# samiwilf/torchrec-oldfork

Hardware: AMD Instinct MI355X
Metric: samples/sec Criteo-1TB DLRM batch 65536 (higher is better)
Workload: dtype f32; 1 GPU; DLRM Criteo-1TB shape: 26 tables (177.9M rows, 84.85 GiB fp32, D=128), 13 dense, pooling factor 1, dense 512-256-128, over 1024-1024-512-256-1, fused exact SGD; global_batch=65536, local_batch=65536, parallelism=mp1: 26 table-wise + 0 row-wise + 0 replicated (data-parallel) tables, dense dp1, ids=uniform, distinct_batches=32, seed=0, data_ranks=1

## Files before the change

### include/tbe_hip.h

```cpp
#ifndef TBE_HIP_H_
#define TBE_HIP_H_

#include <stddef.h>
#include <stdint.h>

#ifdef __cplusplus
extern "C" {
#endif

#define TBE_OK 0
#define TBE_ERR_INVALID_ARGUMENT (-1)
#define TBE_ERR_LAUNCH (-2)
#define TBE_ERR_WORKSPACE (-3)
#define TBE_ERR_UNSUPPORTED (-4)

#define TBE_POOL_SUM 0
#define TBE_POOL_MEAN 1
#define TBE_POOL_NONE 2

#define TBE_OPT_EXACT_SGD 0
#define TBE_OPT_EXACT_ROWWISE_ADAGRAD 1
#define TBE_OPT_ADAM 2
#define TBE_OPT_EXACT_ADAGRAD 3
#define TBE_OPT_DENSE_GRAD 100
// ... 199 lines not shown
                                int32_t B, int32_t D_total, int32_t all_multiple_of_4, void* stream);

int tbe_dlrm_interaction_forward_f32(const float* dense, const float* sparse, int32_t B,
                                     int32_t F, int32_t D, float* out, int64_t out_row_stride,
                                     void* stream);
int tbe_dlrm_interaction_backward_f32(const float* dense, const float* sparse,
                                      const float* grad_out, int64_t grad_row_stride, int32_t B, int32_t F, int32_t D,
                                      float* grad_dense, float* grad_sparse, void* stream);

int tbe_dlrm_interaction_gather_forward_f32(const float* dense, const uint64_t* feat_weights, const int64_t* feat_rows,
                                            const int64_t* feat_window, const int64_t* indices, int32_t B, int32_t F,
                                            int32_t D, float* out, int64_t out_row_stride, int32_t* bounds_errors,
                                            void* stream);
int tbe_dlrm_interaction_gather_backward_f32(const float* dense, const uint64_t* feat_weights, const int64_t* feat_rows,
                                             const int64_t* feat_window, const int64_t* indices, const float* grad_out,
                                             int64_t grad_row_stride, int32_t B, int32_t F, int32_t D, float* grad_dense,
                                             float* grad_sparse, int32_t* bounds_errors, void* stream);

size_t tbe_relu_backward_bias_grad_workspace_bytes(int64_t B, int32_t N);
int tbe_relu_backward_bias_grad_f32(const float* grad_out, const float* act, int64_t B, int32_t N,
                                    float* grad_in, float* bias_grad, void* workspace,
                                    size_t workspace_bytes, void* stream);

size_t tbe_weighted_colsum_workspace_bytes(int64_t B, int32_t N);
int tbe_weighted_colsum_f32(const float* x, const float* w, int64_t B, int32_t N, float* out,
                            void* workspace, size_t workspace_bytes, void* stream);

int64_t tbe_colsum_row_blocks(int64_t B, int32_t N);
int tbe_relu_backward_bias_partials_f32(const float* grad_out, const float* act, int64_t B, int32_t N,
                                        float* grad_in, float* partial, size_t partial_bytes, void* stream);
int tbe_weighted_colsum_partials_f32(const float* x, const float* w, int64_t B, int32_t N, float* partial,
                                     size_t partial_bytes, void* stream);

int tbe_multi_chunk_sum_f32(const int64_t* seg_table, int32_t nseg, int64_t max_numel, float* dst, float scale,
                            void* stream);
int tbe_multi_chunk_sum_host_table_f32(const int64_t* host_seg_table, int32_t nseg, int64_t max_numel, float* dst,
                                       float scale, void* stream);

size_t tbe_bce_with_logits_workspace_bytes(void);
int tbe_bce_with_logits_f32(const float* logits, const void* labels, int32_t label_elem_size, int64_t B, float* loss,
                            float* dlogits, void* workspace, size_t workspace_bytes, void* stream);

int tbe_jagged_2d_to_dense_f32(const float* values, const int64_t* offsets, int32_t B,
                               int32_t D, int32_t max_L, float* dense, void* stream);

int tbe_dense_to_jagged_2d_f32(const float* dense, const int64_t* offsets, int32_t B, int32_t D,
// ... 13 lines not shown
```

### torchrec-oldfork_amd/csrc/mlp_epilogue.hip

```cpp
#include <algorithm>
#include <cstring>

#include "common.hpp"

namespace tbe {

__host__ __device__ inline int rows_per_block(int N) { return N >= 512 ? 256 : 64; }

template <int TX>
__global__ __launch_bounds__(256) void drelu_bgrad_kernel(const float* __restrict__ gy, const float* __restrict__ act,
                                                          float* __restrict__ gx, float* __restrict__ partial,
                                                          int64_t B, int N) {
  constexpr int TY = 256 / TX;
  __shared__ float4 red[TY][TX];
  const int tx = threadIdx.x % TX;
  const int ty = threadIdx.x / TX;
  const int col = (blockIdx.x * TX + tx) * 4;
  const int rpb = rows_per_block(N);
  const int64_t row0 = static_cast<int64_t>(blockIdx.y) * rpb;
  const int64_t row1 = min(B, row0 + rpb);
  float4 acc = make_float4(0.f, 0.f, 0.f, 0.f);
  if (col < N) {
#pragma unroll 4
    for (int64_t r = row0 + ty; r < row1; r += TY) {
// ... 45 lines not shown
      const float s = w[r];
      acc.x = fmaf(s, v.x, acc.x);
      acc.y = fmaf(s, v.y, acc.y);
      acc.z = fmaf(s, v.z, acc.z);
      acc.w = fmaf(s, v.w, acc.w);
    }
  }
  red[ty][tx] = acc;
  __syncthreads();
  if (ty == 0 && col < N) {
    float4 s = red[0][tx];
#pragma unroll
    for (int y = 1; y < TY; ++y) {
      const float4 o = red[y][tx];
      s.x += o.x;
      s.y += o.y;
      s.z += o.z;
      s.w += o.w;
    }
    st4(partial + static_cast<int64_t>(blockIdx.y) * N + col, s);
  }
}

__global__ __launch_bounds__(256) void colsum_partials_kernel(const float* __restrict__ partial, int64_t nblocks, int N,
                                                              float* __restrict__ out) {
  __shared__ float red[4][64];
  const int lane = threadIdx.x & 63;
  const int wave = threadIdx.x >> 6;
  const int c = blockIdx.x * 64 + lane;
  float acc = 0.f;
  if (c < N) {
#pragma unroll 8
    for (int64_t rb = wave; rb < nblocks; rb += 4) acc += partial[rb * N + c];
  }
  red[wave][lane] = acc;
  __syncthreads();
  if (wave == 0 && c < N) out[c] = ((red[0][lane] + red[1][lane]) + red[2][lane]) + red[3][lane];
}

struct ChunkSeg {
  const float* src;
  int64_t chunks;
  int64_t numel;
  int64_t dst_off;
};
constexpr int kChunkSegsByValue = 32;
struct ChunkSegs32 {
  ChunkSeg s[kChunkSegsByValue];
};
__device__ __forceinline__ void multi_chunk_sum_body(const ChunkSeg sg, float* __restrict__ dst, float scale);

__global__ __launch_bounds__(256) void multi_chunk_sum_kernel(const ChunkSeg* __restrict__ segs, float* __restrict__ dst,
                                                              float scale) {
  multi_chunk_sum_body(segs[blockIdx.y], dst, scale);
}
__global__ __launch_bounds__(256) void multi_chunk_sum_args_kernel(const ChunkSegs32 segs, float* __restrict__ dst, float scale) {
  multi_chunk_sum_body(segs.s[blockIdx.y], dst, scale);
}

__device__ __forceinline__ void multi_chunk_sum_body(const ChunkSeg sg, float* __restrict__ dst, float scale) {
// ... 196 lines not shown
  }
  TBE_REQUIRE(x && w && workspace, "tbe_weighted_colsum_f32: null pointer");
  TBE_REQUIRE(((reinterpret_cast<uintptr_t>(x) | reinterpret_cast<uintptr_t>(workspace)) & 15) == 0,
              "tbe_weighted_colsum_f32: tensors must be 16-B aligned");
  TBE_REQUIRE(workspace_bytes >= tbe_weighted_colsum_workspace_bytes(B, N), "tbe_weighted_colsum_f32: workspace too small");
  const int rpb = rows_per_block(N);
  const int64_t nrb = (B + rpb - 1) / rpb;
  TBE_REQUIRE(nrb <= 65535, "tbe_weighted_colsum_f32: B=%lld too large", (long long)B);
  float* partial = static_cast<float*>(workspace);
  const int vecs = N / 4;
  if (vecs >= 64) {
    hipLaunchKernelGGL(wcolsum_kernel<64>, dim3((vecs + 63) / 64, static_cast<unsigned>(nrb)), dim3(256), 0, st, x, w, partial, B, N);
  } else if (vecs >= 32) {
    hipLaunchKernelGGL(wcolsum_kernel<32>, dim3((vecs + 31) / 32, static_cast<unsigned>(nrb)), dim3(256), 0, st, x, w, partial, B, N);
  } else {
    hipLaunchKernelGGL(wcolsum_kernel<16>, dim3((vecs + 15) / 16, static_cast<unsigned>(nrb)), dim3(256), 0, st, x, w, partial, B, N);
  }
  TBE_CHECK_LAUNCH("tbe_weighted_colsum_f32");
  hipLaunchKernelGGL(colsum_partials_kernel, dim3((N + 63) / 64), dim3(256), 0, st, partial, nrb, N, out);
  TBE_CHECK_LAUNCH("tbe_weighted_colsum_f32 colsum");
  return TBE_OK;
}


extern "C" int64_t tbe_colsum_row_blocks(int64_t B, int32_t N) {
  if (B <= 0 || N <= 0) return 0;
  const int rpb = rows_per_block(N);
  return (B + rpb - 1) / rpb;
}

extern "C" int tbe_relu_backward_bias_partials_f32(const float* grad_out, const float* act, int64_t B, int32_t N,
                                                   float* grad_in, float* partial, size_t partial_bytes, void* stream) {
  TBE_REQUIRE(B > 0 && N > 0 && (N & 3) == 0, "tbe_relu_backward_bias_partials_f32: B > 0 and N a positive multiple of 4 required");
  TBE_REQUIRE(grad_out && act && grad_in && partial, "tbe_relu_backward_bias_partials_f32: null pointer");
  TBE_REQUIRE(((reinterpret_cast<uintptr_t>(grad_out) | reinterpret_cast<uintptr_t>(act) |
                reinterpret_cast<uintptr_t>(grad_in) | reinterpret_cast<uintptr_t>(partial)) & 15) == 0,
              "tbe_relu_backward_bias_partials_f32: tensors must be 16-B aligned");
  const int64_t nrb = tbe_colsum_row_blocks(B, N);
  TBE_REQUIRE(nrb <= 65535, "tbe_relu_backward_bias_partials_f32: B=%lld too large", (long long)B);
  TBE_REQUIRE(partial_bytes >= static_cast<size_t>(nrb) * N * sizeof(float), "tbe_relu_backward_bias_partials_f32: partial too small");
  hipStream_t st = static_cast<hipStream_t>(stream);
  const int vecs = N / 4;
  if (vecs >= 64) {
    hipLaunchKernelGGL(drelu_bgrad_kernel<64>, dim3((vecs + 63) / 64, static_cast<unsigned>(nrb)), dim3(256), 0, st, grad_out, act, grad_in, partial, B, N);
  } else if (vecs >= 32) {
    hipLaunchKernelGGL(drelu_bgrad_kernel<32>, dim3((vecs + 31) / 32, static_cast<unsigned>(nrb)), dim3(256), 0, st, grad_out, act, grad_in, partial, B, N);
// ... 83 lines not shown
```

### torchrec-oldfork_amd/fbgemm_gpu/_lib.py

```python
import ctypes
import os
from typing import Optional

import torch

_HERE = os.path.dirname(os.path.abspath(__file__))
LIB_PATH = os.path.normpath(os.path.join(_HERE, "..", "lib", "libtbe_hip.so"))

c_void_p = ctypes.c_void_p
c_i32 = ctypes.c_int32
c_i64 = ctypes.c_int64
c_u64 = ctypes.c_uint64
c_size = ctypes.c_size_t
c_float = ctypes.c_float


class OptimizerArgs(ctypes.Structure):

    _fields_ = [
        ("optimizer", c_i32),
        ("learning_rate", c_float),
        ("eps", c_float),
        ("weight_decay", c_float),
        ("beta1", c_float),
# ... 122 lines not shown
        ctypes.c_int,
        [c_void_p, c_void_p, c_void_p, c_void_p, c_void_p, c_void_p, c_void_p, c_i32, c_i32, c_i32,
         c_i32, c_i32, c_float, c_void_p]),
    "tbe_pooled_exchange_pack": (
        ctypes.c_int,
        [c_void_p, c_void_p, c_void_p, c_void_p, c_void_p, c_void_p, c_void_p, c_i32, c_i32, c_i32,
         c_i32, c_i32, c_float, c_void_p]),
    "tbe_permute_pooled_embs_f32": (
        ctypes.c_int, [c_void_p, c_void_p, c_void_p, c_void_p, c_void_p, c_i32, c_i32, c_i32, c_i32, c_void_p]),
    "tbe_dlrm_interaction_forward_f32": (
        ctypes.c_int, [c_void_p, c_void_p, c_i32, c_i32, c_i32, c_void_p, c_i64, c_void_p]),
    "tbe_dlrm_interaction_backward_f32": (
        ctypes.c_int, [c_void_p, c_void_p, c_void_p, c_i64, c_i32, c_i32, c_i32, c_void_p, c_void_p, c_void_p]),
    "tbe_dlrm_interaction_gather_forward_f32": (
        ctypes.c_int,
        [c_void_p, c_void_p, c_void_p, c_void_p, c_void_p, c_i32, c_i32, c_i32, c_void_p, c_i64, c_void_p, c_void_p]),
    "tbe_dlrm_interaction_gather_backward_f32": (
        ctypes.c_int,
        [c_void_p, c_void_p, c_void_p, c_void_p, c_void_p, c_void_p, c_i64, c_i32, c_i32, c_i32, c_void_p, c_void_p,
         c_void_p, c_void_p]),
    "tbe_relu_backward_bias_grad_workspace_bytes": (c_size, [c_i64, c_i32]),
    "tbe_relu_backward_bias_grad_f32": (
        ctypes.c_int, [c_void_p, c_void_p, c_i64, c_i32, c_void_p, c_void_p, c_void_p, c_size, c_void_p]),
    "tbe_weighted_colsum_workspace_bytes": (c_size, [c_i64, c_i32]),
    "tbe_weighted_colsum_f32": (
        ctypes.c_int, [c_void_p, c_void_p, c_i64, c_i32, c_void_p, c_void_p, c_size, c_void_p]),
    "tbe_colsum_row_blocks": (c_i64, [c_i64, c_i32]),
    "tbe_relu_backward_bias_partials_f32": (
        ctypes.c_int, [c_void_p, c_void_p, c_i64, c_i32, c_void_p, c_void_p, c_size, c_void_p]),
    "tbe_weighted_colsum_partials_f32": (
        ctypes.c_int, [c_void_p, c_void_p, c_i64, c_i32, c_void_p, c_size, c_void_p]),
    "tbe_multi_chunk_sum_f32": (ctypes.c_int, [c_void_p, c_i32, c_i64, c_void_p, c_float, c_void_p]),
    "tbe_multi_chunk_sum_host_table_f32": (ctypes.c_int, [c_void_p, c_i32, c_i64, c_void_p, c_float, c_void_p]),
    "tbe_bce_with_logits_workspace_bytes": (c_size, []),
    "tbe_bce_with_logits_f32": (
        ctypes.c_int, [c_void_p, c_void_p, c_i32, c_i64, c_void_p, c_void_p, c_void_p, c_size, c_void_p]),
    "tbe_jagged_2d_to_dense_f32": (
        ctypes.c_int, [c_void_p, c_void_p, c_i32, c_i32, c_i32, c_void_p, c_void_p]),
    "tbe_dense_to_jagged_2d_f32": (
        ctypes.c_int, [c_void_p, c_void_p, c_i32, c_i32, c_i32, c_i64, c_void_p, c_void_p]),
    "tbe_offsets_range": (ctypes.c_int, [c_void_p, c_i64, c_i64, c_void_p, c_void_p]),
    "tbe_copy_rows": (ctypes.c_int, [c_void_p, c_i64, c_void_p, c_i32, c_i64, c_void_p, c_void_p]),
}

_lib: Optional[ctypes.CDLL] = None

# ... 84 lines not shown
```

### torchrec-oldfork_amd/torchrec_amd/distributed/_device_ops.py

```python
import torch

from fbgemm_gpu import _lib
from fbgemm_gpu._lib import check, ptr, require_gpu, stream_ptr

_def = torch.library.Library("tbe_hip", "DEF")
_def.define("pooled_exchange_unpack(Tensor recv, Tensor feat_out_col, Tensor feat_src, Tensor feat_slab_col, "
            "Tensor slab_offset, Tensor slab_stride, int B_local, int D_total, bool vec, float scale) -> Tensor")
_def.define("pooled_exchange_unpack_into(Tensor recv, Tensor feat_out_col, Tensor feat_src, Tensor feat_slab_col, "
            "Tensor slab_offset, Tensor slab_stride, int B_local, int D_total, bool vec, float scale, Tensor(a!) out) -> Tensor(a!)")
_def.define("pooled_exchange_pack(Tensor grad, Tensor feat_out_col, Tensor feat_src, Tensor feat_slab_col, "
            "Tensor slab_offset, Tensor slab_stride, int numel, bool vec, float scale) -> Tensor")
_def.define("pooled_exchange_pack_into(Tensor grad, Tensor feat_out_col, Tensor feat_src, Tensor feat_slab_col, "
            "Tensor slab_offset, Tensor slab_stride, bool vec, float scale, Tensor(a!) send) -> Tensor(a!)")
_def.define("a2a_pooled_unpack(Tensor recv, Tensor dim_sum_per_rank, int B_local, int D_total, bool vec, float scale) -> Tensor")
_def.define("a2a_pooled_pack(Tensor grad, Tensor dim_sum_per_rank, bool vec, float scale) -> Tensor")
_def.define("relu_backward_bias_grad(Tensor grad_out, Tensor act) -> (Tensor, Tensor)")
_def.define("weighted_colsum(Tensor x, Tensor w) -> Tensor")
_def.define("copy_rows(Tensor src, Tensor rows) -> Tensor")
_def.define("relu_backward_bias_partials(Tensor grad_out, Tensor act) -> (Tensor, Tensor)")
_def.define("weighted_colsum_partials(Tensor x, Tensor w) -> Tensor")
_def.define("multi_chunk_sum(Tensor seg_table, int nseg, int max_numel, Tensor(a!) dst, float scale) -> Tensor(a!)")
_def.define("bce_with_logits(Tensor logits, Tensor labels) -> (Tensor, Tensor)")
_impl = torch.library.Library("tbe_hip", "IMPL", "CUDA")


def _copy_rows(src, rows):
    dev = require_gpu(src, rows)
    if src.dim() != 2 or not src.is_contiguous() or rows.dtype != torch.int32 or rows.dim() != 1:
        raise RuntimeError(f"copy_rows: need a contiguous 2-D src and int32 rows, got {tuple(src.shape)} / {rows.dtype}")
    out = src.new_empty((rows.numel(), src.shape[1]))
    lib = _lib.load()
    with torch.cuda.device(dev):
        check(lib.tbe_copy_rows(ptr(src), src.shape[0], ptr(rows), rows.numel(), src.shape[1] * src.element_size(), ptr(out),
                                stream_ptr(dev)), "tbe_copy_rows")
    return out


def _weighted_colsum(x, w):
    from fbgemm_gpu._lib import workspace
# ... 9 lines not shown
        ws = workspace(lib.tbe_weighted_colsum_workspace_bytes(B, N), dev)
        check(lib.tbe_weighted_colsum_f32(ptr(x), ptr(w), B, N, ptr(out), ptr(ws), ws.numel(), stream_ptr(dev)),
              "tbe_weighted_colsum_f32")
    return out


def _relu_backward_bias_grad(grad_out, act):
    from fbgemm_gpu._lib import workspace

    dev = require_gpu(grad_out, act)
    if grad_out.dim() != 2 or grad_out.shape != act.shape or grad_out.dtype != torch.float32 or act.dtype != torch.float32:
        raise RuntimeError(f"relu_backward_bias_grad: need two float32 [B, N] tensors of one shape, got "
                           f"{tuple(grad_out.shape)} and {tuple(act.shape)}")
    grad_out, act = grad_out.contiguous(), act.contiguous()
    B, N = grad_out.shape
    gx = torch.empty_like(grad_out)
    gb = torch.empty(N, dtype=torch.float32, device=dev)
    lib = _lib.load()
    with torch.cuda.device(dev):
        ws = workspace(lib.tbe_relu_backward_bias_grad_workspace_bytes(B, N), dev)
        check(lib.tbe_relu_backward_bias_grad_f32(ptr(grad_out), ptr(act), B, N, ptr(gx), ptr(gb), ptr(ws), ws.numel(),
                                                  stream_ptr(dev)), "tbe_relu_backward_bias_grad_f32")
    return gx, gb


def _relu_backward_bias_partials(grad_out, act):
    dev = require_gpu(grad_out, act)
    if grad_out.dim() != 2 or grad_out.shape != act.shape or grad_out.dtype != torch.float32 or act.dtype != torch.float32:
        raise RuntimeError(f"relu_backward_bias_partials: need two float32 [B, N] tensors of one shape, got "
                           f"{tuple(grad_out.shape)} and {tuple(act.shape)}")
    grad_out, act = grad_out.contiguous(), act.contiguous()
    B, N = grad_out.shape
    lib = _lib.load()
    gx = torch.empty_like(grad_out)
    partial = torch.empty((lib.tbe_colsum_row_blocks(B, N), N), dtype=torch.float32, device=dev)
    with torch.cuda.device(dev):
        check(lib.tbe_relu_backward_bias_partials_f32(ptr(grad_out), ptr(act), B, N, ptr(gx), ptr(partial),
                                                      partial.numel() * 4, stream_ptr(dev)), "tbe_relu_backward_bias_partials_f32")
    return gx, partial


def _weighted_colsum_partials(x, w):
    dev = require_gpu(x, w)
    if x.dim() != 2 or w.numel() != x.shape[0] or x.dtype != torch.float32 or w.dtype != torch.float32:
        raise RuntimeError(f"weighted_colsum_partials: need float32 x [B, N] and w [B], got {tuple(x.shape)} and {tuple(w.shape)}")
    x, w = x.contiguous(), w.contiguous().view(-1)
# ... 94 lines not shown
        check(_lib.load().tbe_pooled_exchange_pack(
            ptr(grad), ptr(send), ptr(feat_out_col), ptr(feat_src), ptr(feat_slab_col), ptr(slab_offset),
            ptr(slab_stride), feat_src.numel(), slab_offset.numel(), B_local, D_total, int(vec), scale,
            stream_ptr(dev)), "tbe_pooled_exchange_pack")
    return send


def _pack_into(grad, feat_out_col, feat_src, feat_slab_col, slab_offset, slab_stride, vec, scale, send):
    dev = require_gpu(grad, feat_out_col, feat_src, feat_slab_col, slab_offset, slab_stride, send)
    if grad.dim() != 2 or not grad.is_contiguous() or grad.dtype != torch.float32:
        raise RuntimeError("pooled_exchange_pack_into: grad must be a contiguous float32 [B_local, D_total] matrix")
    if send.dtype != torch.float32 or not send.is_contiguous():
        raise RuntimeError("pooled_exchange_pack_into: send must be a contiguous float32 buffer")
    B_local, D_total = grad.shape
    with torch.cuda.device(dev):
        check(_lib.load().tbe_pooled_exchange_pack(
            ptr(grad), ptr(send), ptr(feat_out_col), ptr(feat_src), ptr(feat_slab_col), ptr(slab_offset),
            ptr(slab_stride), feat_src.numel(), slab_offset.numel(), B_local, D_total, int(vec), scale,
            stream_ptr(dev)), "tbe_pooled_exchange_pack")
    return send


_impl.impl("relu_backward_bias_grad", _relu_backward_bias_grad)
_impl.impl("weighted_colsum", _weighted_colsum)
_impl.impl("copy_rows", _copy_rows)
_impl.impl("relu_backward_bias_partials", _relu_backward_bias_partials)
_impl.impl("weighted_colsum_partials", _weighted_colsum_partials)
_impl.impl("multi_chunk_sum", _multi_chunk_sum)
_impl.impl("bce_with_logits", _bce_with_logits)
_impl.impl("pooled_exchange_unpack", _unpack)
_impl.impl("pooled_exchange_unpack_into", _unpack_into)
_impl.impl("pooled_exchange_pack", _pack)
_impl.impl("pooled_exchange_pack_into", _pack_into)
_impl.impl("a2a_pooled_unpack", _simple_unpack)
_impl.impl("a2a_pooled_pack", _simple_pack)
```

### torchrec-oldfork_amd/torchrec_amd/models/dlrm.py

```python
import os
from typing import Dict, List, Optional, Tuple

import torch
from torch import nn

from ..modules.mlp import MLP, LinearOut
from ..profiling import label
from ..sparse.jagged_tensor import KeyedJaggedTensor, KeyedTensor


class SparseArch(nn.Module):

    def __init__(self, embedding_bag_collection: nn.Module) -> None:
        super().__init__()
        self.embedding_bag_collection = embedding_bag_collection
        cfgs = embedding_bag_collection.embedding_bag_configs
        assert cfgs, "Embedding bag collection cannot be empty!"
        self.D: int = cfgs[0].embedding_dim
        self._sparse_feature_names: List[str] = [n for c in cfgs for n in c.feature_names]
        self.F: int = len(self._sparse_feature_names)

    def start(self, features: KeyedJaggedTensor):
        return self.embedding_bag_collection(features)

    def finish(self, pending) -> torch.Tensor:
        sparse_features = pending.wait() if hasattr(pending, "wait") else pending
        B = sparse_features.values().shape[0]
        if sparse_features.keys() == self._sparse_feature_names:
            return sparse_features.values().reshape(B, self.F, self.D)
# ... 154 lines not shown
        self.register_buffer("triu_indices", torch.triu_indices(self.F + 1, self.F + 1, offset=1), persistent=False)

    def forward(self, dense_features: torch.Tensor, sparse_features: torch.Tensor) -> torch.Tensor:
        if self.F <= 0:
            return dense_features
        if self.fused and _fused_interaction_ok(dense_features, sparse_features):
            return _FusedDotInteraction.apply(dense_features, sparse_features, self.pad_rows, self.grad_sinks)
        combined = torch.cat((dense_features.unsqueeze(1), sparse_features), dim=1)
        interactions = torch.bmm(combined, combined.transpose(1, 2))
        flat = interactions[:, self.triu_indices[0], self.triu_indices[1]]
        return torch.cat((dense_features, flat), dim=1)


class OverArch(nn.Module):
    def __init__(self, in_features: int, layer_sizes: List[int], device: Optional[torch.device] = None) -> None:
        super().__init__()
        if len(layer_sizes) <= 1:
            raise ValueError("OverArch must have multiple layers.")
        self.model = nn.Sequential(
            MLP(in_features, layer_sizes[:-1], bias=True, activation="relu", device=device),
            LinearOut(layer_sizes[-2], layer_sizes[-1], bias=True, device=device))

    def forward(self, features: torch.Tensor) -> torch.Tensor:
        return self.model(features)


class DLRM(nn.Module):
    def __init__(self, embedding_bag_collection: nn.Module, dense_in_features: int,
                 dense_arch_layer_sizes: List[int], over_arch_layer_sizes: List[int],
                 dense_device: Optional[torch.device] = None) -> None:
        super().__init__()
        cfgs = embedding_bag_collection.embedding_bag_configs
        assert len(cfgs) > 0, "At least one embedding bag is required"
        D = cfgs[0].embedding_dim
        assert all(c.embedding_dim == D for c in cfgs), "All EmbeddingBagConfigs must have the same dimension"
        if dense_arch_layer_sizes[-1] != D:
            raise ValueError(f"embedding_bag_collection dimension ({D}) and final dense arch layer size "
                             f"({dense_arch_layer_sizes[-1]}) must match.")
        self.sparse_arch = SparseArch(embedding_bag_collection)
        F = self.sparse_arch.F
        self.dense_arch = DenseArch(dense_in_features, dense_arch_layer_sizes, device=dense_device)
        self.inter_arch = InteractionArch(F)
        over_in = D + (F + 1) * F // 2
        self.over_arch = OverArch(over_in, over_arch_layer_sizes, device=dense_device)
        if dense_device is not None:
            self.inter_arch.to(dense_device)
        self.fused_lookup = True
# ... 513 lines not shown
```

### torchrec-oldfork_amd/torchrec_amd/modules/mlp.py

```python
from typing import Callable, List, Optional, Union

import torch
from torch import nn


class _DeferredWgrad:

    pending: Optional[list] = None
    partials_ok: bool = False

    @classmethod
    def compute(cls, gy: torch.Tensor, x: torch.Tensor, c: int) -> torch.Tensor:
        B = x.shape[0]
        if c > 1 and B % c == 0:
            return torch.bmm(gy.view(c, B // c, -1).transpose(1, 2), x.view(c, B // c, -1)).sum(dim=0)
        return gy.t() @ x

    @classmethod
    def compute_partials(cls, gy: torch.Tensor, x: torch.Tensor, c: int) -> torch.Tensor:
        B = x.shape[0]
        if c > 1 and B % c == 0:
            return torch.bmm(gy.view(c, B // c, -1).transpose(1, 2), x.view(c, B // c, -1))
        return (gy.t() @ x).unsqueeze(0)

    @classmethod
    def stashing(cls, t: torch.Tensor) -> bool:
        return cls.pending is not None and t.is_cuda and torch.cuda.is_current_stream_capturing()


class _LinearSplitKWgrad(torch.autograd.Function):

    @staticmethod
    def forward(ctx, x, weight, bias, chunks, fuse_relu):
        ctx.chunks = chunks
        ctx.has_bias = bias is not None
        ctx.fuse_relu = fuse_relu
        ctx.weight_param = weight if (weight.is_leaf and weight.requires_grad) else None
        ctx.bias_param = bias if (bias is not None and bias.is_leaf and bias.requires_grad) else None
        if fuse_relu:
            out = torch._addmm_activation(bias, x, weight.t(), use_gelu=False)
            ctx.save_for_backward(x, weight, out)
            return out
        ctx.save_for_backward(x, weight)
        return torch.nn.functional.linear(x, weight, bias)

    @staticmethod
    def backward(ctx, gy):
        gb = None
        gb_deferred = False
        if ctx.fuse_relu:
            x, weight, out = ctx.saved_tensors
            if ctx.has_bias and gy.dtype == torch.float32 and out.shape[1] % 4 == 0:
                from ..distributed import _device_ops
                if (_DeferredWgrad.partials_ok and ctx.bias_param is not None and ctx.needs_input_grad[2]
                        and _DeferredWgrad.stashing(gy)):
                    gy, part = torch.ops.tbe_hip.relu_backward_bias_partials(gy, out)
                    _DeferredWgrad.pending.append(("p", ctx.bias_param, part))
                    gb_deferred = True
                else:
                    gy, gb = torch.ops.tbe_hip.relu_backward_bias_grad(gy, out)
            else:
                gy = torch.ops.aten.threshold_backward(gy.contiguous(), out, 0.0)
        else:
            x, weight = ctx.saved_tensors
            gy = gy.contiguous()
        gx = None
        if ctx.needs_input_grad[0]:
            if x.dim() == 2 and x.stride(1) == 1 and x.stride(0) > x.shape[1] and x.stride(0) % 4 == 0:
                gx = gy.new_empty((x.shape[0], x.stride(0)))[:, :x.shape[1]]
                torch.mm(gy, weight, out=gx)
            else:
                gx = gy @ weight
        c = ctx.chunks
        w = ctx.weight_param
        if w is not None and ctx.needs_input_grad[1] and _DeferredWgrad.stashing(gy):
            _DeferredWgrad.pending.append(("w", w, gy, x, c))
            gw = None
        else:
            gw = _DeferredWgrad.compute(gy, x, c)
        if gb is None and ctx.has_bias and not gb_deferred:
            gb = gy.sum(dim=0)
        return gx, gw, gb, None, None


class _LinearOneOutput(torch.autograd.Function):

    @staticmethod
    def forward(ctx, x, weight, bias):
        ctx.save_for_backward(x, weight)
        ctx.has_bias = bias is not None
        ctx.weight_param = weight if (weight.is_leaf and weight.requires_grad) else None
        return torch.nn.functional.linear(x, weight, bias)

    @staticmethod
    def backward(ctx, gy):
        from ..distributed import _device_ops

        x, weight = ctx.saved_tensors
        gy = gy.contiguous()
        gx = gy @ weight if ctx.needs_input_grad[0] else None
        if _DeferredWgrad.partials_ok and ctx.weight_param is not None and _DeferredWgrad.stashing(gy):
            part = torch.ops.tbe_hip.weighted_colsum_partials(x, gy.view(-1))
            _DeferredWgrad.pending.append(("p", ctx.weight_param, part.view(part.shape[0], 1, -1)))
            gw = None
        else:
# ... 34 lines not shown
            c = _wgrad_chunks(input.shape[0], self._out_size, self._in_size)
            relu = self._activation_fn is torch.relu and lin.bias is not None
            if c > 1 or relu:
                y = _LinearSplitKWgrad.apply(input, lin.weight, lin.bias, c, relu)
                return y if relu else self._activation_fn(y)
        return self._activation_fn(lin(input))


class MLP(nn.Module):
    def __init__(self, in_size: int, layer_sizes: List[int], bias: bool = True,
                 activation: Union[str, Callable] = torch.relu, device: Optional[torch.device] = None) -> None:
        super().__init__()
        if activation == "relu":
            activation = torch.relu
        elif activation == "sigmoid":
            activation = torch.sigmoid
        sizes = [in_size] + list(layer_sizes)
        self._mlp = nn.Sequential(*[
            Perceptron(sizes[i], sizes[i + 1], bias=bias, activation=activation, device=device)
            for i in range(len(layer_sizes))])

    def forward(self, input: torch.Tensor) -> torch.Tensor:
        return self._mlp(input)
```

Measured before the change: 8.035 million samples/s.

## Fuse ReLU backward with bias/weight gradients for first and final MLP layers

Adds a fused kernel that computes ReLU-masked bias and weight gradients in one pass for layers with small input width (the 13-feature bottom layer). Adds a second kernel that fuses the one-output head with the preceding ReLU layer, producing that layer's input gradient together with the hidden bias, output weight and output bias gradients. Eager backward now gathers weight and bias partials into a single multi-chunk sum. The goal is fewer kernel launches and fewer passes over activations, at the price of more special-case paths that only run outside graph capture.

```diff
diff --git a/include/tbe_hip.h b/include/tbe_hip.h
--- a/include/tbe_hip.h
+++ b/include/tbe_hip.h
@@ -245,6 +245,16 @@
                                     float* grad_in, float* bias_grad, void* workspace,
                                     size_t workspace_bytes, void* stream);
 
+size_t tbe_relu_backward_bias_wgrad_workspace_bytes(int64_t B, int32_t N, int32_t K);
+int tbe_relu_backward_bias_wgrad_f32(const float* grad_out, const float* act, const float* x, int64_t B, int32_t N,
+                                     int32_t K, float* weight_grad, float* bias_grad, void* workspace,
+                                     size_t workspace_bytes, void* stream);
+
+size_t tbe_one_output_relu_backward_workspace_bytes(int64_t B, int32_t N);
+int tbe_one_output_relu_backward_f32(const float* dy, const float* w_out, const float* act, int64_t B, int32_t N,
+                                     float* grad_in, float* bias_grad_hidden, float* weight_grad_out,
+                                     float* bias_grad_out, void* workspace, size_t workspace_bytes, void* stream);
+
 size_t tbe_weighted_colsum_workspace_bytes(int64_t B, int32_t N);
 int tbe_weighted_colsum_f32(const float* x, const float* w, int64_t B, int32_t N, float* out,
                             void* workspace, size_t workspace_bytes, void* stream);
diff --git a/torchrec-oldfork_amd/csrc/mlp_epilogue.hip b/torchrec-oldfork_amd/csrc/mlp_epilogue.hip
--- a/torchrec-oldfork_amd/csrc/mlp_epilogue.hip
+++ b/torchrec-oldfork_amd/csrc/mlp_epilogue.hip
@@ -91,20 +91,209 @@
   }
 }
 
+constexpr int kWgradMaxK = 16;
+template <int TX>
+__global__ __launch_bounds__(256) void drelu_bgrad_wgrad_kernel(const float* __restrict__ gy, const float* __restrict__ act,
+                                                                const float* __restrict__ x, float* __restrict__ partial,
+                                                                int64_t B, int N, int K) {
+  constexpr int TY = 256 / TX;
+  __shared__ float4 red[TY][TX];
+  const int tx = threadIdx.x % TX;
+  const int ty = threadIdx.x / TX;
+  const int col = (blockIdx.x * TX + tx) * 4;
+  const int rpb = rows_per_block(N);
+  const int64_t row0 = static_cast<int64_t>(blockIdx.y) * rpb;
+  const int64_t row1 = min(B, row0 + rpb);
+  float4 bacc = make_float4(0.f, 0.f, 0.f, 0.f);
+  float4 wacc[kWgradMaxK];
+#pragma unroll
+  for (int k = 0; k < kWgradMaxK; ++k) wacc[k] = make_float4(0.f, 0.f, 0.f, 0.f);
+  if (col < N) {
+#pragma unroll 2
+    for (int64_t r = row0 + ty; r < row1; r += TY) {
+      float4 g = ld4(gy + r * N + col);
+      const float4 a = ld4(act + r * N + col);
+      const float* xr = x + r * K;
+      g.x = a.x > 0.f ? g.x : 0.f;
+      g.y = a.y > 0.f ? g.y : 0.f;
+      g.z = a.z > 0.f ? g.z : 0.f;
+      g.w = a.w > 0.f ? g.w : 0.f;
+      bacc.x += g.x;
+      bacc.y += g.y;
+      bacc.z += g.z;
+      bacc.w += g.w;
+#pragma unroll
+      for (int k = 0; k < kWgradMaxK; ++k) {
+        if (k < K) {
+          const float xv = xr[k];
+          wacc[k].x = fmaf(g.x, xv, wacc[k].x);
+          wacc[k].y = fmaf(g.y, xv, wacc[k].y);
+          wacc[k].z = fmaf(g.z, xv, wacc[k].z);
+          wacc[k].w = fmaf(g.w, xv, wacc[k].w);
+        }
+      }
+    }
+  }
+  float* prow = partial + static_cast<int64_t>(blockIdx.y) * (K + 1) * N;
+  auto reduce_store = [&](const float4 v, int j) {
+    red[ty][tx] = v;
+    __syncthreads();
+    if (ty == 0 && col < N) {
+      float4 s = red[0][tx];
+#pragma unroll
+      for (int y = 1; y < TY; ++y) {
+        const float4 o = red[y][tx];
+        s.x += o.x;
+        s.y += o.y;
+        s.z += o.z;
+        s.w += o.w;
+      }
+      st4(prow + static_cast<int64_t>(j) * N + col, s);
+    }
+    __syncthreads();
+  };
+#pragma unroll
+  for (int j = 0; j < kWgradMaxK; ++j) {
+    if (j < K) reduce_store(wacc[j], j);
+  }
+  reduce_store(bacc, K);
+}
+
+template <int TX>
+__global__ __launch_bounds__(256) void one_output_drelu_kernel(const float* __restrict__ dy, const float* __restrict__ w_out,
+                                                               const float* __restrict__ act, float* __restrict__ gx,
+                                                               float* __restrict__ partial, int64_t B, int N) {
+  constexpr int TY = 256 / TX;
+  __shared__ float4 redb[TY][TX];
+  __shared__ float4 redw[TY][TX];
+  __shared__ float redd[TY];
+  const int tx = threadIdx.x % TX;
+  const int ty = threadIdx.x / TX;
+  const int col = (blockIdx.x * TX + tx) * 4;
+  const int rpb = rows_per_block(N);
+  const int64_t row0 = static_cast<int64_t>(blockIdx.y) * rpb;
+  const int64_t row1 = min(B, row0 + rpb);
+  float4 bacc = make_float4(0.f, 0.f, 0.f, 0.f);
+  float4 wacc = make_float4(0.f, 0.f, 0.f, 0.f);
+  float dacc = 0.f;
+  if (col < N) {
+    const float4 wo = ld4(w_out + col);
+#pragma unroll 4
+    for (int64_t r = row0 + ty; r < row1; r += TY) {
+      const float4 a = ld4(act + r * N + col);
+      const float s = dy[r];
+      float4 g;
+      g.x = a.x > 0.f ? s * wo.x : 0.f;
+      g.y = a.y > 0.f ? s * wo.y : 0.f;
+      g.z = a.z > 0.f ? s * wo.z : 0.f;
+      g.w = a.w > 0.f ? s * wo.w : 0.f;
+      st4(gx + r * N + col, g);
+      bacc.x += g.x;
+      bacc.y += g.y;
+      bacc.z += g.z;
+      bacc.w += g.w;
+      wacc.x = fmaf(s, a.x, wacc.x);
+      wacc.y = fmaf(s, a.y, wacc.y);
+      wacc.z = fmaf(s, a.z, wacc.z);
+      wacc.w = fmaf(s, a.w, wacc.w);
+      dacc += s;
+    }
+  }
+  redb[ty][tx] = bacc;
+  redw[ty][tx] = wacc;
+  if (tx == 0) redd[ty] = dacc;
+  __syncthreads();
+  if (ty == 0 && col < N) {
+    float4 sb = redb[0][tx];
+    float4 sw = redw[0][tx];
+#pragma unroll
+    for (int y = 1; y < TY; ++y) {
+      const float4 ob = redb[y][tx];
+      const float4 ow = redw[y][tx];
+      sb.x += ob.x;
+      sb.y += ob.y;
+      sb.z += ob.z;
+      sb.w += ob.w;
+      sw.x += ow.x;
+      sw.y += ow.y;
+      sw.z += ow.z;
+      sw.w += ow.w;
+    }
+    float* prow = partial + static_cast<int64_t>(blockIdx.y) * (2 * N + 4);
+    st4(prow + col, sb);
+    st4(prow + N + col, sw);
+    if (blockIdx.x == 0 && tx == 0) {
+      float sd = redd[0];
+#pragma unroll
+      for (int y = 1; y < TY; ++y) sd += redd[y];
+      prow[2 * N] = sd;
+    }
+  }
+}
+
+__device__ __forceinline__ float colsum_row_blocks(const float* __restrict__ partial, int64_t nblocks, int64_t stride, int64_t c,
+                                                   bool valid, float (*red)[64]) {
+  const int lane = threadIdx.x & 63;
+  const int wave = threadIdx.x >> 6;
+  float acc = 0.f;
+  if (valid) {
+    int64_t rb = wave;
+    for (; rb + 28 < nblocks; rb += 32) {
+      float a[8];
+#pragma unroll
+      for (int u = 0; u < 8; ++u) a[u] = partial[(rb + 4 * u) * stride + c];
+#pragma unroll
+      for (int u = 0; u < 8; ++u) acc += a[u];
+    }
+    for (; rb < nblocks; rb += 4) acc += partial[rb * stride + c];
+  }
+  red[wave][lane] = acc;
+  __syncthreads();
+  return ((red[0][lane] + red[1][lane]) + red[2][lane]) + red[3][lane];
+}
+
 __global__ __launch_bounds__(256) void colsum_partials_kernel(const float* __restrict__ partial, int64_t nblocks, int N,
                                                               float* __restrict__ out) {
   __shared__ float red[4][64];
-  const int lane = threadIdx.x & 63;
-  const int wave = threadIdx.x >> 6;
-  const int c = blockIdx.x * 64 + lane;
-  float acc = 0.f;
-  if (c < N) {
-#pragma unroll 8
-    for (int64_t rb = wave; rb < nblocks; rb += 4) acc += partial[rb * N + c];
-  }
-  red[wave][lane] = acc;
-  __syncthreads();
-  if (wave == 0 && c < N) out[c] = ((red[0][lane] + red[1][lane]) + red[2][lane]) + red[3][lane];
+  const int c = blockIdx.x * 64 + (threadIdx.x & 63);
+  const float s = colsum_row_blocks(partial, nblocks, N, c, c < N, red);
+  if (threadIdx.x < 64 && c < N) out[c] = s;
+}
+
+__global__ __launch_bounds__(256) void wgrad_partials_finish_kernel(const float* __restrict__ partial, int64_t nblocks, int N,
+                                                                    int K, float* __restrict__ weight_grad,
+                                                                    float* __restrict__ bias_grad) {
+  __shared__ float red[4][64];
+  const int W = (K + 1) * N;
+  const int e = blockIdx.x * 64 + (threadIdx.x & 63);
+  const float s = colsum_row_blocks(partial, nblocks, W, e, e < W, red);
+  if (threadIdx.x < 64 && e < W) {
+    const int j = e / N;
+    const int c = e - j * N;
+    if (j < K) {
+      weight_grad[static_cast<int64_t>(c) * K + j] = s;
+    } else {
+      bias_grad[c] = s;
+    }
+  }
+}
+
+__global__ __launch_bounds__(256) void one_output_partials_finish_kernel(const float* __restrict__ partial, int64_t nblocks,
+                                                                         int N, float* __restrict__ bias_grad_hidden,
+                                                                         float* __restrict__ weight_grad_out,
+                                                                         float* __restrict__ bias_grad_out) {
+  __shared__ float red[4][64];
+  const int e = blockIdx.x * 64 + (threadIdx.x & 63);
+  const float s = colsum_row_blocks(partial, nblocks, 2 * N + 4, e, e <= 2 * N, red);
+  if (threadIdx.x < 64 && e <= 2 * N) {
+    if (e < N) {
+      bias_grad_hidden[e] = s;
+    } else if (e < 2 * N) {
+      weight_grad_out[e - N] = s;
+    } else {
+      bias_grad_out[0] = s;
+    }
+  }
 }
 
 struct ChunkSeg {
@@ -347,6 +536,92 @@
   return TBE_OK;
 }
 
+extern "C" size_t tbe_relu_backward_bias_wgrad_workspace_bytes(int64_t B, int32_t N, int32_t K) {
+  if (B <= 0 || N <= 0 || K <= 0) return 256;
+  const int rpb = rows_per_block(N);
+  return align_up(static_cast<size_t>((B + rpb - 1) / rpb) * N * (static_cast<size_t>(K) + 1) * sizeof(float), 256);
+}
+
+extern "C" int tbe_relu_backward_bias_wgrad_f32(const float* grad_out, const float* act, const float* x, int64_t B, int32_t N,
+                                                int32_t K, float* weight_grad, float* bias_grad, void* workspace,
+                                                size_t workspace_bytes, void* stream) {
+  TBE_REQUIRE(B >= 0 && N > 0 && (N & 3) == 0, "tbe_relu_backward_bias_wgrad_f32: N=%d must be a positive multiple of 4", N);
+  TBE_REQUIRE(K >= 1 && K <= kWgradMaxK, "tbe_relu_backward_bias_wgrad_f32: K=%d must be in 1 .. %d", K, kWgradMaxK);
+  TBE_REQUIRE(weight_grad != nullptr && bias_grad != nullptr, "tbe_relu_backward_bias_wgrad_f32: null gradient");
+  hipStream_t st = static_cast<hipStream_t>(stream);
+  if (B == 0) {
+    if (hipMemsetAsync(weight_grad, 0, sizeof(float) * N * K, st) != hipSuccess) return TBE_ERR_LAUNCH;
+    if (hipMemsetAsync(bias_grad, 0, sizeof(float) * N, st) != hipSuccess) return TBE_ERR_LAUNCH;
+    return TBE_OK;
+  }
+  TBE_REQUIRE(grad_out && act && x && workspace, "tbe_relu_backward_bias_wgrad_f32: null pointer");
+  TBE_REQUIRE(((reinterpret_cast<uintptr_t>(grad_out) | reinterpret_cast<uintptr_t>(act) |
+                reinterpret_cast<uintptr_t>(workspace)) & 15) == 0,
+              "tbe_relu_backward_bias_wgrad_f32: grad_out, act and workspace must be 16-B aligned");
+  TBE_REQUIRE(workspace_bytes >= tbe_relu_backward_bias_wgrad_workspace_bytes(B, N, K),
+              "tbe_relu_backward_bias_wgrad_f32: workspace too small");
+  const int rpb = rows_per_block(N);
+  const int64_t nrb = (B + rpb - 1) / rpb;
+  TBE_REQUIRE(nrb <= 65535, "tbe_relu_backward_bias_wgrad_f32: B=%lld too large", (long long)B);
+  float* partial = static_cast<float*>(workspace);
+  const int vecs = N / 4;
+  if (vecs >= 64) {
+    hipLaunchKernelGGL(drelu_bgrad_wgrad_kernel<64>, dim3((vecs + 63) / 64, static_cast<unsigned>(nrb)), dim3(256), 0, st, grad_out, act, x, partial, B, N, K);
+  } else if (vecs >= 32) {
+    hipLaunchKernelGGL(drelu_bgrad_wgrad_kernel<32>, dim3((vecs + 31) / 32, static_cast<unsigned>(nrb)), dim3(256), 0, st, grad_out, act, x, partial, B, N, K);
+  } else {
+    hipLaunchKernelGGL(drelu_bgrad_wgrad_kernel<16>, dim3((vecs + 15) / 16, static_cast<unsigned>(nrb)), dim3(256), 0, st, grad_out, act, x, partial, B, N, K);
+  }
+  TBE_CHECK_LAUNCH("tbe_relu_backward_bias_wgrad_f32");
+  hipLaunchKernelGGL(wgrad_partials_finish_kernel, dim3(((K + 1) * N + 63) / 64), dim3(256), 0, st, partial, nrb, N, K,
+                     weight_grad, bias_grad);
+  TBE_CHECK_LAUNCH("tbe_relu_backward_bias_wgrad_f32 finish");
+  return TBE_OK;
+}
+
+extern "C" size_t tbe_one_output_relu_backward_workspace_bytes(int64_t B, int32_t N) {
+  if (B <= 0 || N <= 0) return 256;
+  const int rpb = rows_per_block(N);
+  return align_up(static_cast<size_t>((B + rpb - 1) / rpb) * (2 * static_cast<size_t>(N) + 4) * sizeof(float), 256);
+}
+
+extern "C" int tbe_one_output_relu_backward_f32(const float* dy, const float* w_out, const float* act, int64_t B, int32_t N,
+                                                float* grad_in, float* bias_grad_hidden, float* weight_grad_out,
+                                                float* bias_grad_out, void* workspace, size_t workspace_bytes, void* stream) {
+  TBE_REQUIRE(B >= 0 && N > 0 && (N & 3) == 0, "tbe_one_output_relu_backward_f32: N=%d must be a positive multiple of 4", N);
+  TBE_REQUIRE(bias_grad_hidden && weight_grad_out && bias_grad_out, "tbe_one_output_relu_backward_f32: null gradient");
+  hipStream_t st = static_cast<hipStream_t>(stream);
+  if (B == 0) {
+    if (hipMemsetAsync(bias_grad_hidden, 0, sizeof(float) * N, st) != hipSuccess) return TBE_ERR_LAUNCH;
+    if (hipMemsetAsync(weight_grad_out, 0, sizeof(float) * N, st) != hipSuccess) return TBE_ERR_LAUNCH;
+    if (hipMemsetAsync(bias_grad_out, 0, sizeof(float), st) != hipSuccess) return TBE_ERR_LAUNCH;
+    return TBE_OK;
+  }
+  TBE_REQUIRE(dy && w_out && act && grad_in && workspace, "tbe_one_output_relu_backward_f32: null pointer");
+  TBE_REQUIRE(((reinterpret_cast<uintptr_t>(w_out) | reinterpret_cast<uintptr_t>(act) | reinterpret_cast<uintptr_t>(grad_in) |
+                reinterpret_cast<uintptr_t>(workspace)) & 15) == 0,
+              "tbe_one_output_relu_backward_f32: w_out, act, grad_in and workspace must be 16-B aligned");
+  TBE_REQUIRE(workspace_bytes >= tbe_one_output_relu_backward_workspace_bytes(B, N),
+              "tbe_one_output_relu_backward_f32: workspace too small");
+  const int rpb = rows_per_block(N);
+  const int64_t nrb = (B + rpb - 1) / rpb;
+  TBE_REQUIRE(nrb <= 65535, "tbe_one_output_relu_backward_f32: B=%lld too large", (long long)B);
+  float* partial = static_cast<float*>(workspace);
+  const int vecs = N / 4;
+  if (vecs >= 64) {
+    hipLaunchKernelGGL(one_output_drelu_kernel<64>, dim3((vecs + 63) / 64, static_cast<unsigned>(nrb)), dim3(256), 0, st, dy, w_out, act, grad_in, partial, B, N);
+  } else if (vecs >= 32) {
+    hipLaunchKernelGGL(one_output_drelu_kernel<32>, dim3((vecs + 31) / 32, static_cast<unsigned>(nrb)), dim3(256), 0, st, dy, w_out, act, grad_in, partial, B, N);
+  } else {
+    hipLaunchKernelGGL(one_output_drelu_kernel<16>, dim3((vecs + 15) / 16, static_cast<unsigned>(nrb)), dim3(256), 0, st, dy, w_out, act, grad_in, partial, B, N);
+  }
+  TBE_CHECK_LAUNCH("tbe_one_output_relu_backward_f32");
+  hipLaunchKernelGGL(one_output_partials_finish_kernel, dim3((2 * N + 1 + 63) / 64), dim3(256), 0, st, partial, nrb, N,
+                     bias_grad_hidden, weight_grad_out, bias_grad_out);
+  TBE_CHECK_LAUNCH("tbe_one_output_relu_backward_f32 finish");
+  return TBE_OK;
+}
+
 
 extern "C" int64_t tbe_colsum_row_blocks(int64_t B, int32_t N) {
   if (B <= 0 || N <= 0) return 0;
diff --git a/torchrec-oldfork_amd/fbgemm_gpu/_lib.py b/torchrec-oldfork_amd/fbgemm_gpu/_lib.py
--- a/torchrec-oldfork_amd/fbgemm_gpu/_lib.py
+++ b/torchrec-oldfork_amd/fbgemm_gpu/_lib.py
@@ -168,6 +168,13 @@
     "tbe_relu_backward_bias_grad_workspace_bytes": (c_size, [c_i64, c_i32]),
     "tbe_relu_backward_bias_grad_f32": (
         ctypes.c_int, [c_void_p, c_void_p, c_i64, c_i32, c_void_p, c_void_p, c_void_p, c_size, c_void_p]),
+    "tbe_relu_backward_bias_wgrad_workspace_bytes": (c_size, [c_i64, c_i32, c_i32]),
+    "tbe_relu_backward_bias_wgrad_f32": (
+        ctypes.c_int, [c_void_p, c_void_p, c_void_p, c_i64, c_i32, c_i32, c_void_p, c_void_p, c_void_p, c_size, c_void_p]),
+    "tbe_one_output_relu_backward_workspace_bytes": (c_size, [c_i64, c_i32]),
+    "tbe_one_output_relu_backward_f32": (
+        ctypes.c_int,
+        [c_void_p, c_void_p, c_void_p, c_i64, c_i32, c_void_p, c_void_p, c_void_p, c_void_p, c_void_p, c_size, c_void_p]),
     "tbe_weighted_colsum_workspace_bytes": (c_size, [c_i64, c_i32]),
     "tbe_weighted_colsum_f32": (
         ctypes.c_int, [c_void_p, c_void_p, c_i64, c_i32, c_void_p, c_void_p, c_size, c_void_p]),
diff --git a/torchrec-oldfork_amd/torchrec_amd/distributed/_device_ops.py b/torchrec-oldfork_amd/torchrec_amd/distributed/_device_ops.py
--- a/torchrec-oldfork_amd/torchrec_amd/distributed/_device_ops.py
+++ b/torchrec-oldfork_amd/torchrec_amd/distributed/_device_ops.py
@@ -1,3 +1,5 @@
+import ctypes
+
 import torch
 
 from fbgemm_gpu import _lib
@@ -15,6 +17,10 @@
 _def.define("a2a_pooled_unpack(Tensor recv, Tensor dim_sum_per_rank, int B_local, int D_total, bool vec, float scale) -> Tensor")
 _def.define("a2a_pooled_pack(Tensor grad, Tensor dim_sum_per_rank, bool vec, float scale) -> Tensor")
 _def.define("relu_backward_bias_grad(Tensor grad_out, Tensor act) -> (Tensor, Tensor)")
+_def.define("relu_backward_bias_wgrad(Tensor grad_out, Tensor act, Tensor x) -> (Tensor, Tensor)")
+_def.define("one_output_relu_backward(Tensor dy, Tensor w_out, Tensor act) -> (Tensor, Tensor, Tensor, Tensor)")
+_def.define("multi_chunk_sum_host(Tensor[] srcs, int[] chunks, int[] numels, int[] dst_offs, Tensor(a!) dst, float scale) "
+            "-> Tensor(a!)")
 _def.define("weighted_colsum(Tensor x, Tensor w) -> Tensor")
 _def.define("copy_rows(Tensor src, Tensor rows) -> Tensor")
 _def.define("relu_backward_bias_partials(Tensor grad_out, Tensor act) -> (Tensor, Tensor)")
@@ -70,6 +76,68 @@
         check(lib.tbe_relu_backward_bias_grad_f32(ptr(grad_out), ptr(act), B, N, ptr(gx), ptr(gb), ptr(ws), ws.numel(),
                                                   stream_ptr(dev)), "tbe_relu_backward_bias_grad_f32")
     return gx, gb
+
+
+def _relu_backward_bias_wgrad(grad_out, act, x):
+    from fbgemm_gpu._lib import workspace
+
+    dev = require_gpu(grad_out, act, x)
+    if (grad_out.dim() != 2 or grad_out.shape != act.shape or x.dim() != 2 or x.shape[0] != grad_out.shape[0]
+            or any(t.dtype != torch.float32 for t in (grad_out, act, x))):
+        raise RuntimeError(f"relu_backward_bias_wgrad: need float32 grad_out / act [B, N] and x [B, K], got "
+                           f"{tuple(grad_out.shape)}, {tuple(act.shape)} and {tuple(x.shape)}")
+    grad_out, act, x = grad_out.contiguous(), act.contiguous(), x.contiguous()
+    B, N = grad_out.shape
+    K = x.shape[1]
+    gw = torch.empty((N, K), dtype=torch.float32, device=dev)
+    gb = torch.empty(N, dtype=torch.float32, device=dev)
+    lib = _lib.load()
+    with torch.cuda.device(dev):
+        ws = workspace(lib.tbe_relu_backward_bias_wgrad_workspace_bytes(B, N, K), dev)
+        check(lib.tbe_relu_backward_bias_wgrad_f32(ptr(grad_out), ptr(act), ptr(x), B, N, K, ptr(gw), ptr(gb), ptr(ws),
+                                                   ws.numel(), stream_ptr(dev)), "tbe_relu_backward_bias_wgrad_f32")
+    return gw, gb
+
+
+def _one_output_relu_backward(dy, w_out, act):
+    from fbgemm_gpu._lib import workspace
+
+    dev = require_gpu(dy, w_out, act)
+    if (act.dim() != 2 or dy.numel() != act.shape[0] or w_out.numel() != act.shape[1]
+            or any(t.dtype != torch.float32 for t in (dy, w_out, act))):
+        raise RuntimeError(f"one_output_relu_backward: need float32 dy [B], w_out [N] and act [B, N], got "
+                           f"{tuple(dy.shape)}, {tuple(w_out.shape)} and {tuple(act.shape)}")
+    dy, w_out, act = dy.contiguous().view(-1), w_out.contiguous().view(-1), act.contiguous()
+    B, N = act.shape
+    gx = torch.empty_like(act)
+    gb_hidden = torch.empty(N, dtype=torch.float32, device=dev)
+    gw_out = torch.empty(N, dtype=torch.float32, device=dev)
+    gb_out = torch.empty(1, dtype=torch.float32, device=dev)
+    lib = _lib.load()
+    with torch.cuda.device(dev):
+        ws = workspace(lib.tbe_one_output_relu_backward_workspace_bytes(B, N), dev)
+        check(lib.tbe_one_output_relu_backward_f32(ptr(dy), ptr(w_out), ptr(act), B, N, ptr(gx), ptr(gb_hidden), ptr(gw_out),
+                                                   ptr(gb_out), ptr(ws), ws.numel(), stream_ptr(dev)),
+              "tbe_one_output_relu_backward_f32")
+    return gx, gb_hidden, gw_out, gb_out
+
+
+def _multi_chunk_sum_host(srcs, chunks, numels, dst_offs, dst, scale):
+    dev = require_gpu(dst, *srcs)
+    n = len(srcs)
+    if not (len(chunks) == len(numels) == len(dst_offs) == n):
+        raise RuntimeError("multi_chunk_sum_host: srcs, chunks, numels and dst_offs must have one length")
+    if dst.dtype != torch.float32 or not dst.is_contiguous():
+        raise RuntimeError("multi_chunk_sum_host: dst must be a contiguous float32 tensor")
+    table = (ctypes.c_int64 * (4 * max(n, 1)))()
+    for s, (src, c, m, off) in enumerate(zip(srcs, chunks, numels, dst_offs)):
+        if src.dtype != torch.float32 or not src.is_contiguous() or src.numel() < c * m or off < 0 or off + m > dst.numel():
+            raise RuntimeError(f"multi_chunk_sum_host: segment {s} does not fit its source or the destination")
+        table[4 * s:4 * s + 4] = [src.data_ptr(), c, m, off]
+    with torch.cuda.device(dev):
+        check(_lib.load().tbe_multi_chunk_sum_host_table_f32(table, n, max(numels, default=0), ptr(dst), scale, stream_ptr(dev)),
+              "tbe_multi_chunk_sum_host_table_f32")
+    return dst
 
 
 def _relu_backward_bias_partials(grad_out, act):
@@ -210,6 +278,9 @@
 
 
 _impl.impl("relu_backward_bias_grad", _relu_backward_bias_grad)
+_impl.impl("relu_backward_bias_wgrad", _relu_backward_bias_wgrad)
+_impl.impl("one_output_relu_backward", _one_output_relu_backward)
+_impl.impl("multi_chunk_sum_host", _multi_chunk_sum_host)
 _impl.impl("weighted_colsum", _weighted_colsum)
 _impl.impl("copy_rows", _copy_rows)
 _impl.impl("relu_backward_bias_partials", _relu_backward_bias_partials)
diff --git a/torchrec-oldfork_amd/torchrec_amd/models/dlrm.py b/torchrec-oldfork_amd/torchrec_amd/models/dlrm.py
--- a/torchrec-oldfork_amd/torchrec_amd/models/dlrm.py
+++ b/torchrec-oldfork_amd/torchrec_amd/models/dlrm.py
@@ -4,7 +4,7 @@
 import torch
 from torch import nn
 
-from ..modules.mlp import MLP, LinearOut
+from ..modules.mlp import MLP, LinearOut, relu_linear_one_output
 from ..profiling import label
 from ..sparse.jagged_tensor import KeyedJaggedTensor, KeyedTensor
 
@@ -205,7 +205,12 @@
             LinearOut(layer_sizes[-2], layer_sizes[-1], bias=True, device=device))
 
     def forward(self, features: torch.Tensor) -> torch.Tensor:
-        return self.model(features)
+        layers = self.model[0]._mlp
+        hidden = features
+        for layer in layers[:-1]:
+            hidden = layer(hidden)
+        logits = relu_linear_one_output(layers[-1], self.model[1], hidden)
+        return logits if logits is not None else self.model[1](layers[-1](hidden))
 
 
 class DLRM(nn.Module):
diff --git a/torchrec-oldfork_amd/torchrec_amd/modules/mlp.py b/torchrec-oldfork_amd/torchrec_amd/modules/mlp.py
--- a/torchrec-oldfork_amd/torchrec_amd/modules/mlp.py
+++ b/torchrec-oldfork_amd/torchrec_amd/modules/mlp.py
@@ -26,6 +26,42 @@
     @classmethod
     def stashing(cls, t: torch.Tensor) -> bool:
         return cls.pending is not None and t.is_cuda and torch.cuda.is_current_stream_capturing()
+
+
+fused_backward_counts = {"first_layer": 0, "one_output": 0, "single_finish": 0}
+
+
+def _capturing(t: torch.Tensor) -> bool:
+    return t.is_cuda and torch.cuda.is_current_stream_capturing()
+
+
+def _finish_wgrad(gy: torch.Tensor, x: torch.Tensor, c: int, bias_part: Optional[torch.Tensor]):
+    out_f, in_f = gy.shape[1], x.shape[1]
+    n = out_f * in_f
+    buf = gy.new_empty(n + (out_f if bias_part is not None else 0))
+    gw = buf[:n].view(out_f, in_f)
+    srcs, chunks, numels, offs = [], [], [], []
+    if c > 1 and x.shape[0] % c == 0:
+        part = _DeferredWgrad.compute_partials(gy, x, c)
+        srcs, chunks, numels, offs = [part], [part.shape[0]], [n], [0]
+    else:
+        torch.mm(gy.t(), x, out=gw)
+    if bias_part is not None:
+        srcs.append(bias_part)
+        chunks.append(bias_part.shape[0])
+        numels.append(out_f)
+        offs.append(n)
+    if srcs:
+        torch.ops.tbe_hip.multi_chunk_sum_host(srcs, chunks, numels, offs, buf, 1.0)
+    return gw, (buf[n:] if bias_part is not None else None)
+
+
+def _input_grad(gy: torch.Tensor, x: torch.Tensor, weight: torch.Tensor) -> torch.Tensor:
+    if x.dim() == 2 and x.stride(1) == 1 and x.stride(0) > x.shape[1] and x.stride(0) % 4 == 0:
+        gx = gy.new_empty((x.shape[0], x.stride(0)))[:, :x.shape[1]]
+        torch.mm(gy, weight, out=gx)
+        return gx
+    return gy @ weight
 
 
 class _LinearSplitKWgrad(torch.autograd.Function):
@@ -48,15 +84,23 @@
     def backward(ctx, gy):
         gb = None
         gb_deferred = False
+        bias_part = None
         if ctx.fuse_relu:
             x, weight, out = ctx.saved_tensors
             if ctx.has_bias and gy.dtype == torch.float32 and out.shape[1] % 4 == 0:
                 from ..distributed import _device_ops
+                eager = gy.is_cuda and x.dtype == torch.float32 and x.dim() == 2 and not _capturing(gy)
+                if eager and not ctx.needs_input_grad[0] and x.shape[1] <= 16 and not _DeferredWgrad.stashing(gy):
+                    gw, gb = torch.ops.tbe_hip.relu_backward_bias_wgrad(gy, out, x)
+                    fused_backward_counts["first_layer"] += 1
+                    return None, gw, gb, None, None
                 if (_DeferredWgrad.partials_ok and ctx.bias_param is not None and ctx.needs_input_grad[2]
                         and _DeferredWgrad.stashing(gy)):
                     gy, part = torch.ops.tbe_hip.relu_backward_bias_partials(gy, out)
                     _DeferredWgrad.pending.append(("p", ctx.bias_param, part))
                     gb_deferred = True
+                elif eager:
+                    gy, bias_part = torch.ops.tbe_hip.relu_backward_bias_partials(gy, out)
                 else:
                     gy, gb = torch.ops.tbe_hip.relu_backward_bias_grad(gy, out)
             else:
@@ -64,16 +108,13 @@
         else:
             x, weight = ctx.saved_tensors
             gy = gy.contiguous()
-        gx = None
-        if ctx.needs_input_grad[0]:
-            if x.dim() == 2 and x.stride(1) == 1 and x.stride(0) > x.shape[1] and x.stride(0) % 4 == 0:
-                gx = gy.new_empty((x.shape[0], x.stride(0)))[:, :x.shape[1]]
-                torch.mm(gy, weight, out=gx)
-            else:
-                gx = gy @ weight
+        gx = _input_grad(gy, x, weight) if ctx.needs_input_grad[0] else None
         c = ctx.chunks
         w = ctx.weight_param
-        if w is not None and ctx.needs_input_grad[1] and _DeferredWgrad.stashing(gy):
+        if bias_part is not None:
+            gw, gb = _finish_wgrad(gy, x, c, bias_part)
+            fused_backward_counts["single_finish"] += 1
+        elif w is not None and ctx.needs_input_grad[1] and _DeferredWgrad.stashing(gy):
             _DeferredWgrad.pending.append(("w", w, gy, x, c))
             gw = None
         else:
@@ -81,6 +122,27 @@
         if gb is None and ctx.has_bias and not gb_deferred:
             gb = gy.sum(dim=0)
         return gx, gw, gb, None, None
+
+
+class _ReluLinearOneOutput(torch.autograd.Function):
+
+    @staticmethod
+    def forward(ctx, x, w_h, b_h, w_o, b_o, chunks):
+        ctx.chunks = chunks
+        act = torch._addmm_activation(b_h, x, w_h.t(), use_gelu=False)
+        ctx.save_for_backward(x, w_h, act, w_o)
+        return torch.nn.functional.linear(act, w_o, b_o)
+
+    @staticmethod
+    def backward(ctx, gy):
+        from ..distributed import _device_ops
+
+        x, w_h, act, w_o = ctx.saved_tensors
+        g, gb_h, gw_o, gb_o = torch.ops.tbe_hip.one_output_relu_backward(gy.contiguous().view(-1), w_o.view(-1), act)
+        gx = _input_grad(g, x, w_h) if ctx.needs_input_grad[0] else None
+        gw_h, _ = _finish_wgrad(g, x, ctx.chunks, None)
+        fused_backward_counts["one_output"] += 1
+        return gx, gw_h, gb_h, gw_o.view(1, -1), gb_o, None
 
 
 class _LinearOneOutput(torch.autograd.Function):
@@ -161,3 +223,15 @@
 
     def forward(self, input: torch.Tensor) -> torch.Tensor:
         return self._mlp(input)
+
+
+def relu_linear_one_output(last: Perceptron, out: nn.Linear, input: torch.Tensor) -> Optional[torch.Tensor]:
+    lin = last._linear
+    params = (lin.weight, lin.bias, out.weight, out.bias)
+    if (last._activation_fn is not torch.relu or out.out_features != 1 or any(p is None for p in params)
+            or lin.out_features % 4 != 0 or not input.is_cuda or input.dim() != 2 or not torch.is_grad_enabled()
+            or any(p.dtype != torch.float32 or not p.requires_grad or not p.is_cuda for p in params)
+            or input.dtype != torch.float32 or torch.cuda.is_current_stream_capturing()):
+        return None
+    c = _wgrad_chunks(input.shape[0], lin.out_features, lin.in_features)
+    return _ReluLinearOneOutput.apply(input, lin.weight, lin.bias, out.weight, out.bias, c)
```

Measured after the change: 7.836 million samples/s. 0.975x the previous value.
